# whabacivch/FL-SLAM

Measured on AMD Instinct MI355X. Metric: LiDAR scans/sec (64k pts, 256 hypotheses) at 1/2/4/8 MI355X, higher is better.
Workload: dtype f64

## Files before the change

fl-slam_amd/csrc/gc_points.hip:

```cpp
#include <hip/hip_runtime.h>
#include <algorithm>
#include <cstdint>
#include <type_traits>
#include "gc_internal.h"
#include "gc_wgla.h"
#include "gc_budget.h"
#include "gc_iobranch_wg.h"
#include "gc_binfin.h"

namespace gc {

typedef double v4d __attribute__((ext_vector_type(4)));

constexpr int NF_COV = 9;
#define GC_RESP_LOAD(ptr) __builtin_nontemporal_load(ptr)

template <int CTRL>
GC_DEV double dpp_f64(double v) {
  const int lo = __builtin_amdgcn_mov_dpp(__double2loint(v), CTRL, 0xF, 0xF, false);
  const int hi = __builtin_amdgcn_mov_dpp(__double2hiint(v), CTRL, 0xF, 0xF, false);
  return __hiloint2double(hi, lo);
}
template <int CTRL>
GC_DEV int dpp_i32(int v) {
  return __builtin_amdgcn_mov_dpp(v, CTRL, 0xF, 0xF, false);
}
constexpr int kDppXor1 = 0xB1, kDppXor2 = 0x4E, kDppHalfMirror = 0x141, kDppMirror = 0x140;

GC_DEV double group16_sum(double v) {
  v += dpp_f64<kDppXor1>(v);
  v += dpp_f64<kDppXor2>(v);
  v += dpp_f64<kDppHalfMirror>(v);
  v += dpp_f64<kDppMirror>(v);
  return v;
}
#ifndef GC_ZSUM
#define GC_ZSUM 0
#endif
template <int XOR>
GC_DEV double swz_f64(double v) {
  constexpr int pat = (XOR << 10) | 0x1F;
  const int lo = __builtin_amdgcn_ds_swizzle(__double2loint(v), pat);
  const int hi = __builtin_amdgcn_ds_swizzle(__double2hiint(v), pat);
  return __hiloint2double(hi, lo);
}
GC_DEV double group16_sum_bins(double v) {
#if GC_ZSUM == 0
  return group16_sum(v);
#else
#if GC_ZSUM == 2
  v += dpp_f64<kDppXor1>(v);
  v += dpp_f64<kDppXor2>(v);
#else
  v += swz_f64<1>(v);
  v += swz_f64<2>(v);
#endif
  v += swz_f64<4>(v);
  v += swz_f64<8>(v);
  return v;
#endif
}
GC_DEV double group16_max(double v) {
  v = fmax(v, dpp_f64<kDppXor1>(v));
  v = fmax(v, dpp_f64<kDppXor2>(v));
  v = fmax(v, dpp_f64<kDppHalfMirror>(v));
  v = fmax(v, dpp_f64<kDppMirror>(v));
  return v;
}
template <int CTRL>
GC_DEV void argmax_step(double& best, int& bidx) {
  const double ob = dpp_f64<CTRL>(best);
  const int oi = dpp_i32<CTRL>(bidx);
  if (ob > best || (ob == best && oi < bidx)) { best = ob; bidx = oi; }
}
GC_DEV void group16_argmax(double& best, int& bidx) {
  argmax_step<kDppXor1>(best, bidx);
  argmax_step<kDppXor2>(best, bidx);
  argmax_step<kDppHalfMirror>(best, bidx);
  argmax_step<kDppMirror>(best, bidx);
}

constexpr int kExpTab = 256;
constexpr double kLn2OverTabHi = 0x1.62e42ffp-9;
constexpr double kLn2OverTabLo = -1.6409824502660487e-13;
constexpr double kTabOverLn2 = 369.3299304675746;
GC_DEV void exp_table_init(double* T) {
  if (threadIdx.x < kExpTab) T[threadIdx.x] = exp2((double)threadIdx.x / kExpTab);
}
constexpr double kRoundMagic = 6755399441055744.0;
GC_DEV double exp_neg(double x, const double* T) {
  const double ks = fma(x, kTabOverLn2, kRoundMagic);
  const double kf = ks - kRoundMagic;
  const int k = __double2loint(ks);
  const double r = fma(-kf, kLn2OverTabLo, fma(-kf, kLn2OverTabHi, x));
  double p = fma(r, 1.0 / 24.0, 1.0 / 6.0);
  p = fma(p, r, 0.5);
  p = fma(p, r, 1.0);
  p = fma(p, r, 1.0);
  return ldexp(T[k & (kExpTab - 1)] * p, k >> 8);
}
template <int N, bool MAGIC = true>
GC_DEV void exp_neg_n(const double (&x)[N], const double* T, double (&out)[N]) {
  double kf[N], tv[N];
  int ki[N];
#pragma unroll
  for (int j = 0; j < N; ++j) {
    if constexpr (MAGIC) {
      const double ks = fma(x[j], kTabOverLn2, kRoundMagic);
      kf[j] = ks - kRoundMagic;
      ki[j] = __double2loint(ks);
    } else {
      kf[j] = rint(x[j] * kTabOverLn2);
      ki[j] = (int)kf[j];
    }
    tv[j] = T[ki[j] & (kExpTab - 1)];
  }
#pragma unroll
  for (int j = 0; j < N; ++j) {
    const double r = fma(-kf[j], kLn2OverTabLo, fma(-kf[j], kLn2OverTabHi, x[j]));
    double p = fma(r, 1.0 / 24.0, 1.0 / 6.0);
    p = fma(p, r, 0.5);
    p = fma(p, r, 1.0);
    p = fma(p, r, 1.0);
    out[j] = ldexp(tv[j] * p, ki[j] >> 8);
  }
}
GC_DEV double recip1(double z) {
  const double r = __builtin_amdgcn_rcp(z);
  return fma(r, fma(-z, r, 1.0), r);
}
GC_DEV double recip(double z) {
  double r = __builtin_amdgcn_rcp(z);
  double e = fma(-z, r, 1.0);
  r = fma(r, e, r);
  e = fma(-z, r, 1.0);
  return fma(r, e, r);
}
template <int HI, int LO>
GC_DEV double vconst() {
  int h, l;
  asm volatile("v_mov_b32 %0, %1" : "=v"(l) : "i"(LO));
  asm volatile("v_mov_b32 %0, %1" : "=v"(h) : "i"(HI));
  return __hiloint2double(h, l);
}
GC_DEV double log_pos(double x) {
  int k;
  double m = frexp(x, &k);
  if (m < 0.70710678118654752440) {
    m *= 2.0;
    --k;
  }
  const double f = m - 1.0;
  const double s = f * recip(2.0 + f);
  const double z = s * s, w = z * z;
  const double t1 = w * (vconst<0x3FD99999, (int)0x9997FA04>() +
                         w * (vconst<0x3FCC71C5, 0x1D8E78AF>() + w * vconst<0x3FC39A09, (int)0xD078C69F>()));
  const double t2 = z * (vconst<0x3FE55555, 0x55555593>() +
                         w * (vconst<0x3FD24924, (int)0x94229359>() +
                              w * (vconst<0x3FC74664, (int)0x96CB03DE>() + w * vconst<0x3FC2F112, (int)0xDF3E5244>())));
  const double R = t2 + t1, hfsq = 0.5 * f * f, dk = (double)k;
  return dk * vconst<0x3FE62E42, (int)0xFEE00000>() -
         ((hfsq - (s * (hfsq + R) + dk * vconst<0x3DEA39EF, 0x35793C76>())) - f);
}
GC_DEV double ent_shift(double inv_tau, int B) {
  asm volatile("" : "+v"(inv_tau), "+v"(B));
  const double ymax = ceil(inv_tau * vconst<0x40A71547, 0x652B82FE>());
  return (ymax * vconst<0x3F362E42, (int)0xFEFA932F>() - (double)B * 1e-12) * 0.25;
}
constexpr int kExpTab2 = 2048;
constexpr double kTab2OverLn2 = 2954.6394437405970;
constexpr double kExp2C1 = 3.3845077175902435e-04;
constexpr double kExp2C2 = kExp2C1 * kExp2C1 * 0.5;
constexpr double kExp2C3 = kExp2C1 * kExp2C1 * kExp2C1 * (1.0 / 6.0);
GC_DEV void exp_table2_init(double* T) {
  for (int j = threadIdx.x; j < kExpTab2; j += blockDim.x) {
    const double v = exp2((double)j / kExpTab2);
    T[j] = __hiloint2double(__double2hiint(v) - (j << 9), __double2loint(v));
  }
}
__device__ __attribute__((aligned(16))) double g_exp_tab2[kExpTab2];
__global__ void __launch_bounds__(256) k_exp_table_init() { exp_table2_init(g_exp_tab2); }
GC_DEV void exp_table2_load(double* T) {
  typedef double dvec2 __attribute__((ext_vector_type(2)));
  for (int j = threadIdx.x; j < kExpTab2 / 2; j += blockDim.x)
    reinterpret_cast<dvec2*>(T)[j] = reinterpret_cast<const dvec2*>(g_exp_tab2)[j];
}
hipError_t init_exp_table(hipStream_t st) {
  hipLaunchKernelGGL(k_exp_table_init, dim3(1), dim3(256), 0, st);
  return hipGetLastError();
}
template <int N>
GC_DEV void exp2s_n(const double (&y)[N], const double* T, double (&out)[N]) {
  double r[N], tv[N];
  int ki[N];
#pragma unroll
  for (int j = 0; j < N; ++j) {
    const double ks = y[j] + kRoundMagic;
    ki[j] = __double2loint(ks);
    r[j] = y[j] - (ks - kRoundMagic);
    tv[j] = T[ki[j] & (kExpTab2 - 1)];
  }
#pragma unroll
  for (int j = 0; j < N; ++j) {
    const double p = fma(fma(fma(kExp2C3, r[j], kExp2C2), r[j], kExp2C1), r[j], 1.0);
    const double t = __hiloint2double(__double2hiint(tv[j]) + (ki[j] << 9), __double2loint(tv[j]));
    out[j] = t * p;
  }
}
template <int N>
GC_DEV void exp2s_shift_n(const double (&y)[N], double Mp, const double* T, double (&out)[N]) {
  double r[N], tv[N];
  int ki[N];
#pragma unroll
  for (int j = 0; j < N; ++j) {
    const double ks = y[j] + Mp;
    ki[j] = __double2loint(ks);
    r[j] = y[j] - (ks - Mp);
    tv[j] = T[ki[j] & (kExpTab2 - 1)];
  }
#pragma unroll
  for (int j = 0; j < N; ++j) {
    const double p = fma(fma(fma(kExp2C3, r[j], kExp2C2), r[j], kExp2C1), r[j], 1.0);
    const double t = __hiloint2double(__double2hiint(tv[j]) + (ki[j] << 9), __double2loint(tv[j]));
    out[j] = t * p;
  }
}
typedef const __attribute__((address_space(3))) char* lds_cptr;
template <int N, unsigned TAB>
GC_DEV void exp2s_shift_tab_n(const double (&y)[N], double Mp, double (&out)[N]) {
  double r[N], tv[N];
  int ki[N];
#pragma unroll
  for (int j = 0; j < N; ++j) {
    const double ks = y[j] + Mp;
    ki[j] = __double2loint(ks);
    r[j] = y[j] - (ks - Mp);
    tv[j] = *reinterpret_cast<const __attribute__((address_space(3))) double*>(
        reinterpret_cast<lds_cptr>((uintptr_t)TAB) + ((unsigned)(ki[j] & (kExpTab2 - 1)) << 3));
  }
#pragma unroll
  for (int j = 0; j < N; ++j) {
    const double p = fma(fma(fma(kExp2C3, r[j], kExp2C2), r[j], kExp2C1), r[j], 1.0);
    const double t = __hiloint2double(__double2hiint(tv[j]) + (ki[j] << 9), __double2loint(tv[j]));
    out[j] = t * p;
  }
}
GC_DEV double sigmoid2(double x, const double* T) {
  const double y[1] = {fmax(-fabs(x), -700.0) * kTab2OverLn2};
  double e[1];
  exp2s_n<1>(y, T, e);
  const double r = recip(1.0 + e[0]);
  return x >= 0.0 ? r : e[0] * r;
}


GC_DEV void lds_wave_sync() {
  __builtin_amdgcn_fence(__ATOMIC_SEQ_CST, "wavefront");
  __builtin_amdgcn_wave_barrier();
}

GC_DEV double sim_nofma(double d0, double d1, double d2, double b0, double b1, double b2) {
#pragma clang fp contract(off)
  double s = d0 * b0 + d1 * b1;
  s = s + d2 * b2;
  return s;
}

GC_DEV void deskew_point_fast(const double* p, double alpha, const double* xi, double* out) {
  const double rho[3] = {alpha * xi[0], alpha * xi[1], alpha * xi[2]};
  const double phi[3] = {alpha * xi[3], alpha * xi[4], alpha * xi[5]};
  const double ts = dot3(phi, phi);
  const double th = sqrt(ts);
  double Bv, Cv, a, b;
  if (th < kSmallAngle) {
    Bv = 0.5 - ts * (1.0 / 24.0);
    Cv = 1.0 / 6.0 - ts * (1.0 / 120.0);
    a = 1.0;
    b = 0.5;
  } else {
    double sn, c;
    sincos(th, &sn, &c);
    const double its = recip((ts < kSmallAngle * kSmallAngle) ? 1.0 : ts);
    const double ith = recip(th);
    Bv = (1.0 - c) * its;
    Cv = (th - sn) * its * ith;
    a = sn * ith;
    b = Bv;
  }
  double V[9], R[9], t[3], q[3];
  rodrigues_form(phi, Bv, Cv, V);
  mat3_vec(V, rho, t);
  rodrigues_form(phi, a, b, R);
  q[0] = p[0] - t[0]; q[1] = p[1] - t[1]; q[2] = p[2] - t[2];
  mat3_tvec(R, q, out);
}
constexpr double kInvFact[22] = {1.0, 1.0, 0.5, 0.16666666666666666, 0.041666666666666664, 0.008333333333333333, 0.001388888888888889, 0.0001984126984126984, 2.48015873015873e-05, 2.7557319223985893e-06, 2.755731922398589e-07, 2.505210838544172e-08, 2.08767569878681e-09, 1.6059043836821613e-10, 1.1470745597729725e-11, 7.647163731819816e-13, 4.779477332387385e-14, 2.8114572543455206e-15, 1.5619206968586225e-16, 8.22063524662433e-18, 4.110317623312165e-19, 1.9572941063391263e-20};
GC_DEV void deskew_point_series(const double* p, double alpha, const double* xi, double* out) {
  const double phi[3] = {alpha * xi[3], alpha * xi[4], alpha * xi[5]};
  const double ts = dot3(phi, phi);
  if (ts > 1.0) {
    deskew_point_fast(p, alpha, xi, out);
    return;
  }
  const double rho[3] = {alpha * xi[0], alpha * xi[1], alpha * xi[2]};
  const double u = -ts;
  double a = kInvFact[19], Bv = kInvFact[20], Cv = kInvFact[21];
#pragma unroll
  for (int k = 8; k >= 0; --k) {
    a = fma(a, u, kInvFact[2 * k + 1]);
    Bv = fma(Bv, u, kInvFact[2 * k + 2]);
    Cv = fma(Cv, u, kInvFact[2 * k + 3]);
  }
  double V[9], R[9], t[3], q[3];
  rodrigues_form(phi, Bv, Cv, V);
  mat3_vec(V, rho, t);
  rodrigues_form(phi, a, Bv, R);
  q[0] = p[0] - t[0]; q[1] = p[1] - t[1]; q[2] = p[2] - t[2];
  mat3_tvec(R, q, out);
}
constexpr double kDeskewShortTs = 0.04;
template <bool SHORT>
GC_DEV void deskew_point_cross(const double* p, double alpha, const double* xi, double* out) {
  const double phi[3] = {alpha * xi[3], alpha * xi[4], alpha * xi[5]};
  const double ts = dot3(phi, phi);
  if (!SHORT && ts > 1.0) {
    deskew_point_fast(p, alpha, xi, out);
    return;
  }
  const double rho[3] = {alpha * xi[0], alpha * xi[1], alpha * xi[2]};
  const double u = -ts;
  constexpr int K = SHORT ? 5 : 9;
  double a = kInvFact[2 * K + 1], Bv = kInvFact[2 * K + 2], Cv = kInvFact[2 * K + 3];
#pragma unroll
  for (int k = K - 1; k >= 0; --k) {
    a = fma(a, u, kInvFact[2 * k + 1]);
    Bv = fma(Bv, u, kInvFact[2 * k + 2]);
    Cv = fma(Cv, u, kInvFact[2 * k + 3]);
  }
  double c1[3], c2[3], q[3];
  cross3(phi, rho, c1);
  cross3(phi, c1, c2);
#pragma unroll
  for (int k = 0; k < 3; ++k) q[k] = p[k] - fma(Cv, c2[k], fma(Bv, c1[k], rho[k]));
  cross3(phi, q, c1);
  cross3(phi, c1, c2);
#pragma unroll
  for (int k = 0; k < 3; ++k) out[k] = fma(Bv, c2[k], fma(-a, c1[k], q[k]));
}
GC_DEV void point_features_w(const double* p, const double* d, double w, double* f) {
  const double wd[3] = {w * d[0], w * d[1], w * d[2]};
  const double wp[3] = {w * p[0], w * p[1], w * p[2]};
  f[0] = w;
  f[1] = wd[0]; f[2] = wd[1]; f[3] = wd[2];
  f[4] = wd[0] * d[0]; f[5] = wd[0] * d[1]; f[6] = wd[0] * d[2];
  f[7] = wd[1] * d[1]; f[8] = wd[1] * d[2]; f[9] = wd[2] * d[2];
  f[10] = wp[0]; f[11] = wp[1]; f[12] = wp[2];
  f[13] = wp[0] * p[0]; f[14] = wp[0] * p[1]; f[15] = wp[0] * p[2];
  f[16] = wp[1] * p[1]; f[17] = wp[1] * p[2]; f[18] = wp[2] * p[2];
}
GC_DEV void direction_fast(const double* p, const double* o, double eps, double* d) {
  const double r0 = p[0] - o[0], r1 = p[1] - o[1], r2 = p[2] - o[2];
  const double inv = recip(sqrt(r0 * r0 + r1 * r1 + r2 * r2) + eps);
  d[0] = r0 * inv; d[1] = r1 * inv; d[2] = r2 * inv;
}
GC_DEV double sigmoid_fast(double x, const double* T) {
  const double e = exp_neg(fmax(-fabs(x), -800.0), T);
  const double r = recip(1.0 + e);
  return x >= 0.0 ? r : e * r;
}
GC_DEV double window_weight_fast(double t, double t0, double t1, double inv_sig, const double* T) {
  const double wr = sigmoid_fast((t - t0) * inv_sig, T) * sigmoid_fast((t1 - t) * inv_sig, T);
  return wr * (1.0 - 1e-12) + 1e-12;
}

GC_DEV double window_weight2(double t, double t0, double t1, double inv_sig, const double* T) {
  const double wr = sigmoid2((t - t0) * inv_sig, T) * sigmoid2((t1 - t) * inv_sig, T);
  return wr * (1.0 - 1e-12) + 1e-12;
}

GC_DEV void point_features(const double* p, const double* d, double w, double* f) {
  f[0] = w;
  f[1] = w * d[0]; f[2] = w * d[1]; f[3] = w * d[2];
  f[4] = w * (d[0] * d[0]); f[5] = w * (d[0] * d[1]); f[6] = w * (d[0] * d[2]);
  f[7] = w * (d[1] * d[1]); f[8] = w * (d[1] * d[2]); f[9] = w * (d[2] * d[2]);
  f[10] = w * p[0]; f[11] = w * p[1]; f[12] = w * p[2];
  f[13] = w * (p[0] * p[0]); f[14] = w * (p[0] * p[1]); f[15] = w * (p[0] * p[2]);
  f[16] = w * (p[1] * p[1]); f[17] = w * (p[1] * p[2]); f[18] = w * (p[2] * p[2]);
}


__global__ void __launch_bounds__(256) k_budget_partials(const double* __restrict__ w, int64_t n_in,
                                                         int64_t stride, double* part) {
  __shared__ double red[4];
  budget_partial_block(w, n_in, stride, blockIdx.x, part, red);
}

__global__ void k_budget_final(const double* __restrict__ part, int64_t n_in, int64_t n_cap, int64_t stride,
// ... 662 lines not shown
  double* Tx = lds + fused_tab_offset(BPL);
  const double ysc = A.inv_tau * kTab2OverLn2;
  constexpr int NACC = 1;
  v4d acc4[NACC][BPL];
  double accx[BPL][NX];
#pragma unroll
  for (int j = 0; j < BPL; ++j) {
    acc4[0][j] = v4d{0.0, 0.0, 0.0, 0.0};
    acc4[NACC - 1][j] = v4d{0.0, 0.0, 0.0, 0.0};
#pragma unroll
    for (int t = 0; t < NX; ++t) accx[j][t] = 0.0;
  }
  double sumw = 0.0, entq = 0.0, mxr = 0.0;
  double zst = 1.0;
  int zex = 0;
  const double ymax = ceil(ysc);
  const double Mp = kRoundMagic - ymax;
  const double Beps = (double)B * 1e-12;
  double np[3] = {0.0, 0.0, 0.0}, ntt = 0.0, nww = 0.0;
  auto fetch = [&](int it2) {
    const int64_t j = chunk0 + (int64_t)it2 * 256 + wv * 64 + lane;
    np[0] = 0.0; np[1] = 0.0; np[2] = 0.0; ntt = 0.0; nww = 0.0;
    if (j < n_cap && j < n_sel) {
      const int64_t i = j * stride;
      np[0] = pts_raw[3 * i]; np[1] = pts_raw[3 * i + 1]; np[2] = pts_raw[3 * i + 2];
      ntt = t_raw[i];
      nww = PRE ? A.w_win[j] : w_raw[i];
    }
  };
  {
    const bool ok = ta.ok;
    np[0] = ok ? ta.np[0] : 0.0; np[1] = ok ? ta.np[1] : 0.0; np[2] = ok ? ta.np[2] : 0.0;
    ntt = ok ? ta.ntt : 0.0; nww = ok ? ta.nww : 0.0;
  }
  unsigned next = 0;
  constexpr int NQ = NB / 4;
  const int cq = lane & 3;
  double bq[NQ][3];
#pragma unroll
  for (int k = 0; k < NQ; ++k) {
    const int b = min(NQ * cq + k, B - 1);
#pragma unroll
    for (int r = 0; r < 3; ++r) bq[k][r] = A.bins[3 * b + r] * ysc;
  }
  auto run_iters = [&](auto pad_tag) {
    constexpr bool PAD = decltype(pad_tag)::value;
    for (int it = 0; it < iters; ++it) {
      const int64_t wbase = chunk0 + (int64_t)it * 256 + wv * 64;
      if (ctr && !late_next && it == iters - 1 && threadIdx.x == 0) next = atomicAdd(ctr, 1u);
      double d[3];
      {
        const bool inr = !PAD || wbase + lane < n_cap;
        double p[3] = {np[0], np[1], np[2]};
        const double tt = ntt, ww = nww * scale;
        if (it + 1 < iters) fetch(it + 1);
        const double al = (tt - t0) * inv_denom;
        const double ph[3] = {al * xr[3], al * xr[4], al * xr[5]};
        double q[3];
        if (__all(dot3(ph, ph) <= kDeskewShortTs)) deskew_point_cross<true>(p, al, xr, q);
        else deskew_point_cross<false>(p, al, xr, q);
        const double wd = inr ? (PRE ? ww : ww * window_weight2(tt, t0, t1, inv_sig, Tx)) : 0.0;
        direction_fast(q, o, 1e-12, d);
        sumw += wd;
        double f[NF];
        point_features_w(q, d, wd, f);
#pragma unroll
        for (int k = 0; k < NF; ++k)
          if (k != DF) F[(k < DF ? k : k - 1) * FS + lane] = f[k];
      }
#pragma unroll
      for (int sk = 0; sk < 4; ++sk) {
        const int pt = 16 * sk + (lane >> 2);
        const double dx = __shfl(d[0], pt), dy = __shfl(d[1], pt), dz = __shfl(d[2], pt);
        const double vf = (!PAD || wbase + pt < n_cap) ? 1.0 : 0.0;
        double e[NQ];
        double Zl = 0.0, sl = 0.0, em = 0.0;
#pragma unroll
        for (int k0 = 0; k0 < NQ; k0 += 4) {
          double x[4], ex[4];
#pragma unroll
          for (int kk = 0; kk < 4; ++kk) {
            const int k = k0 + kk;
            x[kk] = fma(dz, bq[k][2], fma(dy, bq[k][1], dx * bq[k][0]));
          }
          exp2s_shift_tab_n<4, TAB>(x, Mp, ex);
#pragma unroll
          for (int kk = 0; kk < 4; ++kk) {
            const int k = k0 + kk;
            e[k] = (FULL || NQ * cq + k < B) ? ex[kk] : 0.0;
            Zl += e[k];
            sl = fma(e[k], x[kk], sl);
            em = fmax(em, e[k]);
          }
        }
        double Z = Zl + dpp_f64<kDppXor1>(Zl);
        Z = Z + dpp_f64<kDppXor2>(Z);
        const double rZ = recip1(Z);
        entq = fma(sl * rZ, vf, entq);
        mxr = fmax(mxr, em * rZ * vf);
        if (cq == 0) zst *= PAD ? fma(Z - 1.0, vf, 1.0) : Z;
        {
          double* er = E + (lane >> 2) * ES + NQ * cq;
#pragma unroll
          for (int k = 0; k < NQ; k += 2) *reinterpret_cast<dvec2*>(er + k) = dvec2{e[k] * rZ, e[k + 1] * rZ};
        }
        lds_wave_sync();
#pragma unroll
        for (int s = 0; s < 4; ++s) {
          const int ss = 4 * sk + s;
          const int pl = 4 * ss + g;
          const double fb = F[bl * FS + pl];
          double fk[NX];
#pragma unroll
          for (int t = 0; t < NX; ++t) fk[t] = F[(16 + t) * FS + pl];
#pragma unroll
          for (int j = 0; j < BPL; ++j) {
            const double a = E[(4 * s + g) * ES + 16 * j + bl];
            acc4[ss % NACC][j] = __builtin_amdgcn_mfma_f64_16x16x4f64(a, fb, acc4[ss % NACC][j], 0, 0, 0);
#pragma unroll
            for (int t = 0; t < NX; ++t) accx[j][t] = fma(a, fk[t], accx[j][t]);
          }
        }
        lds_wave_sync();
      }
      int e8;
      zst = frexp(zst, &e8);
      zex += e8;
    }
  };
  if (chunk0 + (int64_t)iters * 256 <= n_cap) run_iters(std::false_type{});
  else run_iters(std::true_type{});
  int64_t npts = n_cap - chunk0;
  npts = npts < 0 ? 0 : (npts > (int64_t)iters * 256 ? (int64_t)iters * 256 : npts);
  const double logacc = log_pos(zst) + (double)zex * 0.69314718055994530942;
  const double ent = logacc - entq * kExp2C1 + ((lane == 0) ? (ymax * kExp2C1 - Beps) * (double)npts * 0.25 : 0.0);
#pragma unroll
  for (int j = 0; j < BPL; ++j)
    if (NACC == 2) acc4[0][j] += acc4[NACC - 1][j];
  if (ahead) ahead->valid = false;
  if (ctr && late_next && threadIdx.x == 0) *late_next = atomicAdd(ctr, 1u);
  const auto pre = [&]() {
    if (ctr && !late_next && threadIdx.x == 0) *task_slot = next;
  };
  const auto mid = [&]() {
    if (!ctr || late_next) return;
    const unsigned tn = *task_slot;
    ahead->t = tn;
    if (tn < T) task_operands<PRE>(A, (int)(tn % (unsigned)Hl), (int64_t)(tn / (unsigned)Hl), n_sel, stride, *ahead);
  };
  write_partial_record_mfma<BPL, NX, DF, FULL, WD>(acc4[0], accx, ent, mxr, sumw, (double)npts, B, lds, rec, pre, mid);
  __syncthreads();
}

template <int BPL, bool FULL, bool PRE, bool SEL_CHECK = false>
GC_DEV void bins_task(const FusedArgs& A, int h, int64_t c, double* lds, double* rec, unsigned* ctr,
                      unsigned* task_slot, TaskAhead* ahead, unsigned T, int Hl, unsigned* late_next, int bt_task,
                      int64_t n_sel, int64_t stride) {
  (void)bt_task;
  if constexpr (SEL_CHECK)
    if (n_sel < 0) selection_of(A, &n_sel, &stride);
  if constexpr (bins_lp(BPL)) {
    bins_task_lp<BPL, FULL, PRE>(A, h, c, lds, rec, ctr, task_slot, ahead, T, Hl, late_next, n_sel, stride);
    return;
  }
  constexpr int NF = NF_BASE;
  constexpr int DF = 9;
  constexpr int NX = NF - 16 - 1;
  constexpr int NS = kFusedNS;
  const int64_t n_cap = A.n_cap;
  const int B = A.B;
  int iters;
  const int64_t chunk0 = chunk_first(A, c, &iters);
  const int lane = threadIdx.x & 63, wv = threadIdx.x >> 6;
  const int g = lane >> 4, bl = lane & 15;
  const int fcol = bl >= DF ? bl + 1 : bl;
  double* F = lds + wv * (NS * kFusedFS);
  const double o[3] = {A.o0, A.o1, A.o2};
  TaskAhead ta_local;
  TaskAhead& ta = ahead ? *ahead : ta_local;
  if (!ahead || !ahead->valid) task_operands<PRE>(A, h, c, n_sel, stride, ta);
  double xr[6];
#pragma unroll
  for (int k = 0; k < 6; ++k) xr[k] = ta.xr[k];
  const double* __restrict__ pts_raw = A.pts_raw;
  const double* __restrict__ t_raw = A.t_raw;
  const double* __restrict__ w_raw = A.w_raw;
  const double t0 = A.t0, t1 = A.t1;
  const double scale = A.bscal[2];
  const double denom = fmax(t1 - t0, 1e-12);
  const double inv_denom = 1.0 / denom;
  const double inv_sig = 1.0 / fmax(0.1 * denom, 1e-6);
  double* Tx = lds + 4 * kFusedFS * NS;
  double* Lb = Tx + kExpTab2;
  const double ysc = A.inv_tau * kTab2OverLn2;
  constexpr int NACC = kFusedNacc;
  v4d acc4[NACC][BPL];
  double accx[BPL][NX];
#pragma unroll
  for (int j = 0; j < BPL; ++j) {
    acc4[0][j] = v4d{0.0, 0.0, 0.0, 0.0};
    acc4[NACC - 1][j] = v4d{0.0, 0.0, 0.0, 0.0};
#pragma unroll
    for (int t = 0; t < NX; ++t) accx[j][t] = 0.0;
  }
  double sumw = 0.0, entq = 0.0, mxr = 0.0;
  double zst = 1.0;
  int zex = 0;
  const double ymax = ceil(ysc);
  const double Mp = kRoundMagic - ymax;
  double np[3] = {0.0, 0.0, 0.0}, ntt = 0.0, nww = 0.0;
  auto fetch = [&](int it2) {
    const int64_t j = chunk0 + (int64_t)it2 * 256 + wv * 64 + lane;
    np[0] = 0.0; np[1] = 0.0; np[2] = 0.0; ntt = 0.0; nww = 0.0;
    if (j < n_cap && j < n_sel) {
      const int64_t i = j * stride;
      np[0] = pts_raw[3 * i]; np[1] = pts_raw[3 * i + 1]; np[2] = pts_raw[3 * i + 2];
      ntt = t_raw[i];
      nww = PRE ? A.w_win[j] : w_raw[i];
    }
  };
  {
    const bool ok = ta.ok;
    np[0] = ok ? ta.np[0] : 0.0; np[1] = ok ? ta.np[1] : 0.0; np[2] = ok ? ta.np[2] : 0.0;
    ntt = ok ? ta.ntt : 0.0; nww = ok ? ta.nww : 0.0;
  }
  unsigned next = 0;
  auto run_iters = [&](auto pad_tag) {
    constexpr bool PAD = decltype(pad_tag)::value;
    for (int it = 0; it < iters; ++it) {
      const int64_t wbase = chunk0 + (int64_t)it * 256 + wv * 64;
      if (ctr && !late_next && it == iters - 1 && threadIdx.x == 0) next = atomicAdd(ctr, 1u);
      {
        const int64_t j = wbase + lane;
        const bool inr = j < n_cap;
        double p[3] = {np[0], np[1], np[2]};
        const double tt = ntt, ww = nww * scale;
        if (it + 1 < iters) fetch(it + 1);
        double q[3], d[3], f[NF];
        const double al = (tt - t0) * inv_denom;
        {
          const double ph[3] = {al * xr[3], al * xr[4], al * xr[5]};
          if (__all(dot3(ph, ph) <= kDeskewShortTs)) deskew_point_cross<true>(p, al, xr, q);
          else deskew_point_cross<false>(p, al, xr, q);
        }
        const double wd = inr ? (PRE ? ww : ww * window_weight2(tt, t0, t1, inv_sig, Tx)) : 0.0;
        direction_fast(q, o, 1e-12, d);
        point_features_w(q, d, wd, f);
        sumw += wd;
  #pragma unroll
        for (int k = 0; k < NF; ++k)
          if (k != DF) F[k * kFusedFS + lane] = f[k];
        F[(NF + 0) * kFusedFS + lane] = d[0];
        F[(NF + 1) * kFusedFS + lane] = d[1];
        F[(NF + 2) * kFusedFS + lane] = d[2];
        F[(NF + 3) * kFusedFS + lane] = inr ? 1.0 : 0.0;
      }
      lds_wave_sync();
      for (int s8 = 0; s8 < 16; s8 += kFusedUnr) {
  #pragma unroll
      for (int s = s8; s < s8 + kFusedUnr; ++s) {
        const int pl = s * 4 + g;
        const double d0 = F[(NF + 0) * kFusedFS + pl], d1 = F[(NF + 1) * kFusedFS + pl], d2 = F[(NF + 2) * kFusedFS + pl];
        const double vf = PAD ? F[(NF + 3) * kFusedFS + pl] : 1.0;
        const double fb = F[fcol * kFusedFS + pl];
        double e[BPL], x[BPL], ex[BPL];
  #pragma unroll
        for (int j = 0; j < BPL; ++j) {
          const int b = bl + 16 * j;
          x[j] = fma(d0, Lb[b], fma(d1, Lb[64 + b], d2 * Lb[128 + b]));
        }
        exp2s_shift_tab_n<BPL, 8u * 4u * kFusedFS * kFusedNS>(x, Mp, ex);
  #pragma unroll
        for (int j = 0; j < BPL; ++j) e[j] = (FULL || bl + 16 * j < B) ? ex[j] : 0.0;
        double zl = e[0];
  #pragma unroll
        for (int j = 1; j < BPL; ++j) zl += e[j];
        const double Z = group16_sum_bins(zl);
        const double rZ = recip1(Z);
        double r[BPL];
  #pragma unroll
        for (int j = 0; j < BPL; ++j) r[j] = e[j] * rZ;
        double rm = r[0];
  #pragma unroll
        for (int j = 1; j < BPL; ++j) rm = fmax(rm, r[j]);
  #pragma unroll
        for (int j = 0; j < BPL; ++j)
          entq = fma(r[j] * vf, x[j], entq);
        mxr = fmax(mxr, rm * vf);
        zst *= PAD ? fma(Z - 1.0, vf, 1.0) : Z;
  #pragma unroll
        for (int j = 0; j < BPL; ++j)
          acc4[s % NACC][j] = __builtin_amdgcn_mfma_f64_16x16x4f64(r[j], fb, acc4[s % NACC][j], 0, 0, 0);
  #pragma unroll
        for (int t = 0; t < NX; ++t) {
          const double fk = F[(17 + t) * kFusedFS + pl];
  #pragma unroll
          for (int j = 0; j < BPL; ++j) accx[j][t] = fma(r[j], fk, accx[j][t]);
        }
      }
        int e8;
        zst = frexp(zst, &e8);
        zex += e8;
      }
      lds_wave_sync();
#ifdef GC_BINS_TIMING
      if (it == 0 && threadIdx.x == 0 && bt_task >= 0 && bt_task < 16384) g_task_ep[2 * bt_task] = GC_BT_NOW();
#endif
    }
  };
  if (chunk0 + (int64_t)iters * 256 <= n_cap) run_iters(std::false_type{});
  else run_iters(std::true_type{});
#ifdef GC_BINS_TIMING
  if (threadIdx.x == 0 && bt_task >= 0 && bt_task < 16384) g_task_ep[2 * bt_task + 1] = GC_BT_NOW();
  if ((threadIdx.x & 63) == 0 && bt_task >= 0 && bt_task < 16384) g_task_wv[4 * bt_task + (threadIdx.x >> 6)] = GC_BT_NOW();
#endif
  int64_t npts = n_cap - chunk0;
  npts = npts < 0 ? 0 : (npts > (int64_t)iters * 256 ? (int64_t)iters * 256 : npts);
  const double logacc = log_pos(zst) + (double)zex * 0.69314718055994530942;
  const double ent = (bl == 0 ? logacc : 0.0) - entq * kExp2C1 +
                     ((lane == 0) ? ent_shift(A.inv_tau, B) * (double)npts : 0.0);
#pragma unroll
  for (int j = 0; j < BPL; ++j)
    if (NACC == 2) acc4[0][j] += acc4[NACC - 1][j];
  if (ahead) ahead->valid = false;
  if (ctr && late_next && threadIdx.x == 0) *late_next = atomicAdd(ctr, 1u);
  const auto pre = [&]() {
    if (ctr && !late_next && threadIdx.x == 0) *task_slot = next;
  };
  const auto mid = [&]() {
    if (!ctr || late_next) return;
    const unsigned tn = *task_slot;
    ahead->t = tn;
    if (tn < T) task_operands<PRE>(A, (int)(tn % (unsigned)Hl), (int64_t)(tn / (unsigned)Hl), n_sel, stride, *ahead);
  };
  write_partial_record_mfma<BPL, NX, DF, FULL, NS * kFusedFS>(acc4[0], accx, ent, mxr, sumw, (double)npts, B, lds, rec, pre, mid);
  __syncthreads();
}

template <int BPL, bool FULL, bool AHEAD>
__global__ void __launch_bounds__(256, kFusedOcc) k_bins_io(FusedArgs A, PipeDev P, ScanArgs S,
                                                             const double* __restrict__ odom, int n_io, int io_on,
                                                             int H, int64_t chunks, unsigned* ctr) {
  extern __shared__ double lds[];
  unsigned& task_s = *reinterpret_cast<unsigned*>(lds + fused_lds_doubles(A.B));
#ifdef GC_BINS_TIMING
  const double bt0 = GC_BT_NOW();
  double bt1 = bt0;
  int bt_n = 0;
#endif
  if ((int)blockIdx.x < n_io) {
    lpred_wg(P, S, blockIdx.x, lds);
    if (io_on) io_branch_wg(P, S, odom, blockIdx.x, lds);
#ifdef GC_BINS_TIMING
    if (threadIdx.x == 0 && blockIdx.x < 8192) {
      double* g = g_bins_trace + 4 * blockIdx.x;
      g[0] = bt0; g[1] = bt0; g[2] = GC_BT_NOW(); g[3] = -1.0;
    }
#endif
    return;
  }
  bins_prologue<BPL>(A, lds);
#ifdef GC_BINS_TIMING
  bt1 = GC_BT_NOW();
#endif
  const int RL = A.B * NF_BASE + REC_EXTRA;
  const unsigned T = (unsigned)(H * chunks);
  if (threadIdx.x == 0) task_s = atomicAdd(ctr, 1u);
  __syncthreads();
  TaskAhead ahead;
  ahead.valid = false;
  ahead.ok = false;
  ahead.t = task_s;
  int64_t n_sel, stride;
  selection_of(A, &n_sel, &stride);
  if constexpr (AHEAD) {
    n_sel = uniform_i64(n_sel);
    stride = uniform_i64(stride);
  }
  for (;;) {
    const unsigned t = __builtin_amdgcn_readfirstlane(ahead.t);
    if (t >= T) break;
    const int64_t c = t / H;
    const int h = t % H;
#ifdef GC_BINS_TIMING
    const double tt0 = GC_BT_NOW();
#endif
    if constexpr (AHEAD) {
      bins_task<BPL, FULL, true>(A, h, c, lds, A.partials + ((int64_t)h * chunks + c) * RL, ctr, &task_s, &ahead, T, H,
                                 nullptr, (int)t, n_sel, stride);
    } else {
      unsigned next = 0;
      bins_task<BPL, FULL, true, true>(A, h, c, lds, A.partials + ((int64_t)h * chunks + c) * RL, ctr, &task_s, &ahead, T,
                                 H, &next, (int)t, n_sel, stride);
      if (threadIdx.x == 0) task_s = next;
      __syncthreads();
      ahead.t = task_s;
    }
#ifdef GC_BINS_TIMING
    ++bt_n;
    if (threadIdx.x == 0 && t < 16384) {
      unsigned xcc = 0;
      asm volatile("s_getreg_b32 %0, hwreg(HW_REG_XCC_ID)" : "=s"(xcc));
      double* g = g_task_trace + 4 * t;
      g[0] = tt0; g[1] = GC_BT_NOW(); g[2] = (double)blockIdx.x; g[3] = (double)(xcc & 0xf);
    }
#endif
  }
#ifdef GC_BINS_TIMING
  if (threadIdx.x == 0 && blockIdx.x < 8192) {
    double* g = g_bins_trace + 4 * blockIdx.x;
    g[0] = bt0; g[1] = bt1; g[2] = GC_BT_NOW(); g[3] = (double)bt_n;
  }
#endif
}

template <int BPL, bool FULL>
__global__ void __launch_bounds__(256, kFusedOcc) k_bins_fused(FusedArgs A) {
  extern __shared__ double lds[];
  bins_prologue<BPL>(A, lds);
  const int RL = A.B * NF_BASE + REC_EXTRA;
  int64_t n_sel, stride;
  selection_of(A, &n_sel, &stride);
  bins_task<BPL, FULL, false>(A, blockIdx.y, blockIdx.x, lds,
                       A.partials + ((int64_t)blockIdx.y * gridDim.x + blockIdx.x) * RL, nullptr, nullptr, nullptr,
                       0u, 1, nullptr, -1, n_sel, stride);
}

constexpr int kFinWG = 1024;
GC_DEV void finalize_hyp(int h, int B, int NF, int64_t chunks, const double* __restrict__ partials, double eps_psd,
                         double eps_mass, double* stats, double* cert, double* sm) {
  const int RL = B * NF + REC_EXTRA;
  const double* P = partials + (int64_t)h * chunks * RL;
  const int imax = B * NF + 1;
  if (RL <= kFinWG) finalize_reduce<1, 32>(P, RL, imax, chunks, sm);
  else finalize_reduce<2, 16>(P, RL, imax, chunks, sm);
  __syncthreads();
  double Nl = 0.0, N2l = 0.0, psdl = 0.0, epsl = 0.0, sfl = 0.0;
  if ((int)threadIdx.x < B) {
    const int b = threadIdx.x;
    const double N = sm[b * NF];
    finalize_bin(sm + b * NF, NF, eps_psd, eps_mass, stats + ((int64_t)h * B + b) * GC_BIN_STATS, &psdl, &epsl);
    Nl = N; N2l = N * N; sfl = N / (N + eps_mass);
  }
  if (threadIdx.x >= 64) return;
  const double Nt = wave_sum(Nl);
  const double N2 = wave_sum(N2l);
  const double psd = wave_sum(psdl);
  const double mer = wave_max(epsl);
  const double sf = wave_sum(sfl);
  if (threadIdx.x == 0) {
    const double* ex = sm + B * NF;
    double* c = cert + (int64_t)h * GC_BIN_CERT;
    c[0] = Nt * Nt / (N2 + eps_mass);
    c[1] = sf / (double)B;
    c[2] = psd;
    c[3] = mer;
    c[4] = ex[0] / (ex[3] + eps_mass);
    c[5] = ex[1];
    c[6] = ex[2];
    c[7] = psd + mer;
  }
}
__global__ void __launch_bounds__(kFinWG) k_bins_finalize(int B, int NF, int64_t chunks,
                                                       const double* __restrict__ partials,
                                                       double eps_psd, double eps_mass,
                                                       double* stats, double* cert) {
  extern __shared__ double sm[];
  finalize_hyp(blockIdx.x, B, NF, chunks, partials, eps_psd, eps_mass, stats, cert, sm);
}

constexpr int kFinBins = 6;
#ifndef GC_FIN_KU
#define GC_FIN_KU 16
#endif
constexpr int kFinSplitWG = 128;
#ifndef GC_FOLD_CHUNKS
#define GC_FOLD_CHUNKS 32
#endif
constexpr int64_t kFoldChunks = GC_FOLD_CHUNKS;
static_assert(kFinBins * NF_BASE + REC_EXTRA <= kFinSplitWG, "one lane per record entry");
__global__ void __launch_bounds__(kFinSplitWG) k_bins_finalize_split(int B, int NF, int64_t chunks,
                                                                     const double* __restrict__ partials,
                                                                     double eps_psd, double eps_mass, double* stats,
                                                                     double* cert, double* aux, int64_t* done_word,
                                                                     int64_t ticket) {
  __shared__ double sm[kFinBins * NF_BASE + REC_EXTRA];
  if (done_word && blockIdx.x == 0 && blockIdx.y == 0 && threadIdx.x == 0)
    __hip_atomic_store(done_word, ticket, __ATOMIC_RELAXED, __HIP_MEMORY_SCOPE_SYSTEM);
  const int h = blockIdx.y, s = blockIdx.x;
  const int RL = B * NF + REC_EXTRA;
  const int b0 = s * kFinBins, nb = min(kFinBins, B - b0);
  const bool last = s == (int)gridDim.x - 1;
  const int ne = nb * NF + (last ? REC_EXTRA : 0);
  const int e0 = b0 * NF, imax = B * NF + 1;
  const double* P = partials + (int64_t)h * chunks * RL;
  const int t = threadIdx.x;
  if (t < ne) {
    const int e = e0 + t;
    constexpr int KU = GC_FIN_KU;
    double v = 0.0;
    for (int64_t c = 0; c < chunks; c += KU) {
      double x[KU];
#pragma unroll
      for (int u = 0; u < KU; ++u) x[u] = c + u < chunks ? P[(c + u) * RL + e] : 0.0;
#pragma unroll
      for (int u = 0; u < KU; ++u) v = e == imax ? fmax(v, x[u]) : v + x[u];
    }
    sm[t] = v;
  }
  __syncthreads();
  if (t < nb) {
    double* ax = aux + ((int64_t)h * B + b0 + t) * 2;
    finalize_bin(sm + t * NF, NF, eps_psd, eps_mass, stats + ((int64_t)h * B + b0 + t) * GC_BIN_STATS, ax, ax + 1);
  } else if (last && t == 64) {
    const double* ex = sm + nb * NF;
    double* c = cert + (int64_t)h * GC_BIN_CERT;
    c[4] = ex[0] / (ex[3] + eps_mass);
    c[5] = ex[1];
    c[6] = ex[2];
  }
}

__global__ void k_kappa(int64_t n, const double* __restrict__ R, double eps_r, double d, double r0,
                        double tau, double* out) {
  const int64_t i = (int64_t)blockIdx.x * blockDim.x + threadIdx.x;
  if (i < n) out[i] = kappa_blend(R[i], eps_r, d, r0, tau);
}

__global__ void k_psd3(int batch, const double* __restrict__ M, double eps, double* Mo, double* cert) {
  const int i = blockIdx.x * blockDim.x + threadIdx.x;
  if (i >= batch) return;
  double A[9], P[9], c[6];
  for (int k = 0; k < 9; ++k) A[k] = M[9 * i + k];
  psd_project3(A, eps, P, c);
  for (int k = 0; k < 9; ++k) Mo[9 * i + k] = P[k];
  for (int k = 0; k < 6; ++k) cert[6 * i + k] = c[k];
}

__global__ void __launch_bounds__(256) k_psd_wg(int d, const double* __restrict__ M, double eps,
                                                double* Mo, double* cert) {
  __shared__ double Ml[kDZ * kDZ], Mp[kDZ * kDZ], scr[2 * kDZ * kDZ + 4 * kDZ], red[4], c6[6];
  const int i = blockIdx.x;
  for (int k = threadIdx.x; k < d * d; k += kWG) Ml[k] = M[(int64_t)i * d * d + k];
  __syncthreads();
  wg_psd_project(Ml, Mp, eps, d, scr, red, c6);
  for (int k = threadIdx.x; k < d * d; k += kWG) Mo[(int64_t)i * d * d + k] = Mp[k];
  if (threadIdx.x < 6) cert[6 * i + threadIdx.x] = c6[threadIdx.x];
}

__host__ __device__ inline int psd_ws_len(int dp) { return 3 * dp * dp + 4 * dp + 8; }
__global__ void __launch_bounds__(256) k_psd_any(int d, const double* __restrict__ M, double eps, double* Mo,
                                                 double* cert, double* gws) {
  extern __shared__ double lds_psd[];
  const int dp = d + (d & 1);
  const int64_t i = blockIdx.x;
  double* A = gws ? gws + i * psd_ws_len(dp) : lds_psd;
  double* V = A + dp * dp;
  double* Ms = V + dp * dp;
  double* w = Ms + dp * dp;
  double* cs = w + dp;
  double* red = cs + 3 * dp;
  const double* Mi = M + i * d * d;
  double symloc = 0.0;
  for (int idx = threadIdx.x; idx < dp * dp; idx += kWG) {
    const int r = idx / dp, c = idx % dp;
    double sv = 0.0;
    if (r < d && c < d) {
      sv = 0.5 * (Mi[r * d + c] + Mi[c * d + r]);
      const double dd = sv - Mi[r * d + c];
      symloc += dd * dd;
    }
    A[idx] = sv;
    Ms[idx] = sv;
  }
  __syncthreads();
  const double symd = wg_sum(symloc, red);
  wg_jacobi_eigh(A, V, w, dp, cs, red);
  double mnl = 1e308, mxl = -1e308, nnl = 0.0;
// ... 404 lines not shown
```

Measured before the change: 867.0.

## Batch softmax normalizer reductions across points with transposed DPP sum

```diff
diff --git a/fl-slam_amd/csrc/gc_points.hip b/fl-slam_amd/csrc/gc_points.hip
--- a/fl-slam_amd/csrc/gc_points.hip
+++ b/fl-slam_amd/csrc/gc_points.hip
@@ -35,8 +35,12 @@
   return v;
 }
 #ifndef GC_ZSUM
-#define GC_ZSUM 0
-#endif
+#define GC_ZSUM 4
+#endif
+#ifndef GC_ZSUM_AHEAD
+#define GC_ZSUM_AHEAD GC_ZSUM
+#endif
+constexpr int kZsumBatched = 3, kZsumBatched2 = 4;
 template <int XOR>
 GC_DEV double swz_f64(double v) {
   constexpr int pat = (XOR << 10) | 0x1F;
@@ -44,21 +48,22 @@
   const int hi = __builtin_amdgcn_ds_swizzle(__double2hiint(v), pat);
   return __hiloint2double(hi, lo);
 }
+template <int MODE>
 GC_DEV double group16_sum_bins(double v) {
-#if GC_ZSUM == 0
-  return group16_sum(v);
-#else
-#if GC_ZSUM == 2
-  v += dpp_f64<kDppXor1>(v);
-  v += dpp_f64<kDppXor2>(v);
-#else
-  v += swz_f64<1>(v);
-  v += swz_f64<2>(v);
-#endif
-  v += swz_f64<4>(v);
-  v += swz_f64<8>(v);
-  return v;
-#endif
+  if constexpr (MODE == 1 || MODE == 2) {
+    if constexpr (MODE == 2) {
+      v += dpp_f64<kDppXor1>(v);
+      v += dpp_f64<kDppXor2>(v);
+    } else {
+      v += swz_f64<1>(v);
+      v += swz_f64<2>(v);
+    }
+    v += swz_f64<4>(v);
+    v += swz_f64<8>(v);
+    return v;
+  } else {
+    return group16_sum(v);
+  }
 }
 GC_DEV double group16_max(double v) {
   v = fmax(v, dpp_f64<kDppXor1>(v));
@@ -136,6 +141,40 @@
   e = fma(-z, r, 1.0);
   return fma(r, e, r);
 }
+constexpr int kDppRowShl4 = 0x104, kDppRowShl8 = 0x108, kDppRowBcast0 = 0x150;
+template <int CTRL>
+GC_DEV double dpp_f64_z(double v) {
+  const int lo = __builtin_amdgcn_update_dpp(0, __double2loint(v), CTRL, 0xF, 0xF, true);
+  const int hi = __builtin_amdgcn_update_dpp(0, __double2hiint(v), CTRL, 0xF, 0xF, true);
+  return __hiloint2double(hi, lo);
+}
+template <int LANE>
+GC_DEV double row_bcast_f64(double v) {
+  return __builtin_amdgcn_update_dpp(0.0, v, kDppRowBcast0 + LANE, 0xF, 0xF, true);
+}
+GC_DEV void group16_sum4(const double (&z)[4], int lane, double (&Z)[4], double (&rZ)[4]) {
+  const bool b0 = (lane & 1) != 0, b1 = (lane & 2) != 0;
+  const double a01 = (b0 ? z[1] : z[0]) + dpp_f64<kDppXor1>(b0 ? z[0] : z[1]);
+  const double a23 = (b0 ? z[3] : z[2]) + dpp_f64<kDppXor1>(b0 ? z[2] : z[3]);
+  double q = (b1 ? a23 : a01) + dpp_f64<kDppXor2>(b1 ? a01 : a23);
+  q += dpp_f64_z<kDppRowShl4>(q);
+  q += dpp_f64_z<kDppRowShl8>(q);
+  const double rq = recip1(q);
+  Z[0] = row_bcast_f64<0>(q); rZ[0] = row_bcast_f64<0>(rq);
+  Z[1] = row_bcast_f64<1>(q); rZ[1] = row_bcast_f64<1>(rq);
+  Z[2] = row_bcast_f64<2>(q); rZ[2] = row_bcast_f64<2>(rq);
+  Z[3] = row_bcast_f64<3>(q); rZ[3] = row_bcast_f64<3>(rq);
+}
+GC_DEV void group16_sum2(const double (&z)[2], int lane, double (&Z)[2], double (&rZ)[2]) {
+  const bool b0 = (lane & 1) != 0;
+  double q = (b0 ? z[1] : z[0]) + dpp_f64<kDppXor1>(b0 ? z[0] : z[1]);
+  q += dpp_f64<kDppXor2>(q);
+  q += dpp_f64_z<kDppRowShl4>(q);
+  q += dpp_f64_z<kDppRowShl8>(q);
+  const double rq = recip1(q);
+  Z[0] = row_bcast_f64<0>(q); rZ[0] = row_bcast_f64<0>(rq);
+  Z[1] = row_bcast_f64<1>(q); rZ[1] = row_bcast_f64<1>(rq);
+}
 template <int HI, int LO>
 GC_DEV double vconst() {
   int h, l;
@@ -243,6 +282,24 @@
     const double p = fma(fma(fma(kExp2C3, r[j], kExp2C2), r[j], kExp2C1), r[j], 1.0);
     const double t = __hiloint2double(__double2hiint(tv[j]) + (ki[j] << 9), __double2loint(tv[j]));
     out[j] = t * p;
+  }
+}
+template <int N, unsigned TAB>
+GC_DEV void exp2s_shift_tab_tp_n(const double (&y)[N], double Mp, double (&t)[N], double (&p)[N]) {
+  double r[N], tv[N];
+  int ki[N];
+#pragma unroll
+  for (int j = 0; j < N; ++j) {
+    const double ks = y[j] + Mp;
+    ki[j] = __double2loint(ks);
+    r[j] = y[j] - (ks - Mp);
+    tv[j] = *reinterpret_cast<const __attribute__((address_space(3))) double*>(
+        reinterpret_cast<lds_cptr>((uintptr_t)TAB) + ((unsigned)(ki[j] & (kExpTab2 - 1)) << 3));
+  }
+#pragma unroll
+  for (int j = 0; j < N; ++j) {
+    p[j] = fma(fma(fma(kExp2C3, r[j], kExp2C2), r[j], kExp2C1), r[j], 1.0);
+    t[j] = __hiloint2double(__double2hiint(tv[j]) + (ki[j] << 9), __double2loint(tv[j]));
   }
 }
 GC_DEV double sigmoid2(double x, const double* T) {
@@ -1211,13 +1268,13 @@
   __syncthreads();
 }
 
-template <int BPL, bool FULL, bool PRE, bool SEL_CHECK = false>
+template <int BPL, bool FULL, bool PRE, int ZMODE>
 GC_DEV void bins_task(const FusedArgs& A, int h, int64_t c, double* lds, double* rec, unsigned* ctr,
                       unsigned* task_slot, TaskAhead* ahead, unsigned T, int Hl, unsigned* late_next, int bt_task,
                       int64_t n_sel, int64_t stride) {
   (void)bt_task;
-  if constexpr (SEL_CHECK)
-    if (n_sel < 0) selection_of(A, &n_sel, &stride);
+  constexpr int ZB = FULL && BPL == 1 ? 1 : ZMODE == kZsumBatched ? 4 : ZMODE == kZsumBatched2 ? 2 : 1;
+  static_assert(kFusedUnr % ZB == 0, "the unrolled block holds whole batches");
   if constexpr (bins_lp(BPL)) {
     bins_task_lp<BPL, FULL, PRE>(A, h, c, lds, rec, ctr, task_slot, ahead, T, Hl, late_next, n_sel, stride);
     return;
@@ -1316,6 +1373,7 @@
       }
       lds_wave_sync();
       for (int s8 = 0; s8 < 16; s8 += kFusedUnr) {
+        if constexpr (ZB == 1) {
   #pragma unroll
       for (int s = s8; s < s8 + kFusedUnr; ++s) {
         const int pl = s * 4 + g;
@@ -1334,7 +1392,7 @@
         double zl = e[0];
   #pragma unroll
         for (int j = 1; j < BPL; ++j) zl += e[j];
-        const double Z = group16_sum_bins(zl);
+        const double Z = group16_sum_bins<ZMODE>(zl);
         const double rZ = recip1(Z);
         double r[BPL];
   #pragma unroll
@@ -1357,6 +1415,63 @@
           for (int j = 0; j < BPL; ++j) accx[j][t] = fma(r[j], fk, accx[j][t]);
         }
       }
+        } else {
+  #pragma unroll
+      for (int sb = s8; sb < s8 + kFusedUnr; sb += ZB) {
+        double e[ZB][BPL], x[ZB][BPL], zl[ZB], Z[ZB], rZ[ZB];
+  #pragma unroll
+        for (int u = 0; u < ZB; ++u) {
+          const int pl = (sb + u) * 4 + g;
+          const double d0 = F[(NF + 0) * kFusedFS + pl], d1 = F[(NF + 1) * kFusedFS + pl], d2 = F[(NF + 2) * kFusedFS + pl];
+          double et[BPL], ep[BPL];
+  #pragma unroll
+          for (int j = 0; j < BPL; ++j) {
+            const int b = bl + 16 * j;
+            x[u][j] = fma(d0, Lb[b], fma(d1, Lb[64 + b], d2 * Lb[128 + b]));
+          }
+          exp2s_shift_tab_tp_n<BPL, 8u * 4u * kFusedFS * kFusedNS>(x[u], Mp, et, ep);
+  #pragma unroll
+          for (int j = 0; j < BPL; ++j) e[u][j] = (FULL || bl + 16 * j < B) ? et[j] * ep[j] : 0.0;
+          if constexpr (FULL && BPL > 1) {
+            zl[u] = fma(et[0], ep[0], e[u][1]);
+  #pragma unroll
+            for (int j = 2; j < BPL; ++j) zl[u] = fma(et[j], ep[j], zl[u]);
+          } else {
+            zl[u] = e[u][0];
+  #pragma unroll
+            for (int j = 1; j < BPL; ++j) zl[u] += e[u][j];
+          }
+        }
+        if constexpr (ZB == 4) group16_sum4(zl, lane, Z, rZ);
+        else group16_sum2(zl, lane, Z, rZ);
+  #pragma unroll
+        for (int u = 0; u < ZB; ++u) {
+          const int s = sb + u;
+          const int pl = s * 4 + g;
+          const double vf = PAD ? F[(NF + 3) * kFusedFS + pl] : 1.0;
+          const double fb = F[fcol * kFusedFS + pl];
+          double r[BPL];
+  #pragma unroll
+          for (int j = 0; j < BPL; ++j) r[j] = e[u][j] * rZ[u];
+          double rm = r[0];
+  #pragma unroll
+          for (int j = 1; j < BPL; ++j) rm = fmax(rm, r[j]);
+  #pragma unroll
+          for (int j = 0; j < BPL; ++j) entq = fma(r[j] * vf, x[u][j], entq);
+          mxr = fmax(mxr, rm * vf);
+          zst *= PAD ? fma(Z[u] - 1.0, vf, 1.0) : Z[u];
+  #pragma unroll
+          for (int j = 0; j < BPL; ++j)
+            acc4[s % NACC][j] = __builtin_amdgcn_mfma_f64_16x16x4f64(r[j], fb, acc4[s % NACC][j], 0, 0, 0);
+  #pragma unroll
+          for (int t = 0; t < NX; ++t) {
+            const double fk = F[(17 + t) * kFusedFS + pl];
+  #pragma unroll
+            for (int j = 0; j < BPL; ++j) accx[j][t] = fma(r[j], fk, accx[j][t]);
+          }
+        }
+      }
+        }
         int e8;
         zst = frexp(zst, &e8);
         zex += e8;
@@ -1445,12 +1560,12 @@
     const double tt0 = GC_BT_NOW();
 #endif
     if constexpr (AHEAD) {
-      bins_task<BPL, FULL, true>(A, h, c, lds, A.partials + ((int64_t)h * chunks + c) * RL, ctr, &task_s, &ahead, T, H,
-                                 nullptr, (int)t, n_sel, stride);
+      bins_task<BPL, FULL, true, GC_ZSUM_AHEAD>(A, h, c, lds, A.partials + ((int64_t)h * chunks + c) * RL, ctr, &task_s,
+                                                &ahead, T, H, nullptr, (int)t, n_sel, stride);
     } else {
       unsigned next = 0;
-      bins_task<BPL, FULL, true, true>(A, h, c, lds, A.partials + ((int64_t)h * chunks + c) * RL, ctr, &task_s, &ahead, T,
-                                 H, &next, (int)t, n_sel, stride);
+      bins_task<BPL, FULL, true, GC_ZSUM>(A, h, c, lds, A.partials + ((int64_t)h * chunks + c) * RL, ctr, &task_s, &ahead,
+                                          T, H, &next, (int)t, n_sel, stride);
       if (threadIdx.x == 0) task_s = next;
       __syncthreads();
       ahead.t = task_s;
@@ -1480,9 +1595,9 @@
   const int RL = A.B * NF_BASE + REC_EXTRA;
   int64_t n_sel, stride;
   selection_of(A, &n_sel, &stride);
-  bins_task<BPL, FULL, false>(A, blockIdx.y, blockIdx.x, lds,
-                       A.partials + ((int64_t)blockIdx.y * gridDim.x + blockIdx.x) * RL, nullptr, nullptr, nullptr,
-                       0u, 1, nullptr, -1, n_sel, stride);
+  bins_task<BPL, FULL, false, GC_ZSUM>(A, blockIdx.y, blockIdx.x, lds,
+                                A.partials + ((int64_t)blockIdx.y * gridDim.x + blockIdx.x) * RL, nullptr, nullptr,
+                                nullptr, 0u, 1, nullptr, -1, n_sel, stride);
 }
 
 constexpr int kFinWG = 1024;
```

Measured after the change: 882.5 (median of 6 runs). 1.8% higher.
